# tyb311/TCCT

Measured on AMD Instinct MI355X. Metric: OCT B-scans/sec fwd+bwd(+clip+AdamW), stc_tt bs=8 1x800x1100, higher is better.
Workload: dtype bf16; 1 GPU; stc_tt --los=di bs=8/GPU 1x800x1100 (net tensors 3x800x1104); global_batch=8, parallelism=dp1, ranks=1, grad_allreduce=none, slowest_step=88

## Files before the change

### include/tcct_hip.h

```cpp
#ifndef TCCT_HIP_H
#define TCCT_HIP_H
#include <stdint.h>
#ifdef __cplusplus
extern "C" {
#endif

typedef void* tcct_stream_t;

enum { TCCT_F32 = 0, TCCT_BF16 = 1 };
enum { TCCT_ACT_NONE = 0, TCCT_ACT_LRELU = 1, TCCT_ACT_HSWISH = 2, TCCT_ACT_GELU = 3, TCCT_ACT_SIGMOID = 4,
       TCCT_ACT_ABS = 5 };
enum { TCCT_CRIT_DICE = 0, TCCT_CRIT_DICE2 = 1, TCCT_CRIT_IOU = 2, TCCT_CRIT_MSE = 3 };
enum { TCCT_MCRIT_DICE = 0, TCCT_MCRIT_DICE2 = 1, TCCT_MCRIT_IOU = 2, TCCT_MCRIT_CE = 3 };

int tcct_version(void);
const char* tcct_last_error(void);
int tcct_set_outputs_prezeroed(int on);

int tcct_image_to_nhwc4(const float* img, void* out, int N, int Csrc, int H, int Wsrc, int Wdst, int dtype,
                        tcct_stream_t stream);
int tcct_u8_gather2d(const uint8_t* src, uint8_t* dst, int N, int SH, int SW, int C, int sy0, int sx0, int sh, int sw, int DH, int DW,
                     int dy0, int dx0, int dh, int dw, int flipy, int flipx, int mul, int div, int fill, tcct_stream_t stream);
int tcct_onehot_to_index(const int64_t* onehot, uint8_t* lab, int N, int C, int64_t HW, tcct_stream_t stream);
int tcct_labels_to_u8(const int64_t* lab, uint8_t* out, int N, int H, int Wsrc, int Wdst, tcct_stream_t stream);
// ... 59 lines not shown
                           int pre_act, int act, int dtype, tcct_stream_t stream);
int tcct_bn2_add_act_bwd_reduce(const void* xa, const void* xb, const void* dy, int64_t M, int C, const float* mean_rstdA,
                                const float* abA, const float* mean_rstdB, const float* abB, int pre_act, int act, double* sums,
                                int dtype, tcct_stream_t stream);
int tcct_bn2_add_act_bwd_apply(const void* xa, const void* xb, const void* dy, void* dxa, void* dxb, int64_t M, int C,
                               const float* mean_rstdA, const float* abA, const float* mean_rstdB, const float* abB,
                               const double* sums, int pre_act, int act, float* dgammaA, float* dbetaA, float* dgammaB,
                               float* dbetaB, int dtype, tcct_stream_t stream);

int tcct_layernorm_fwd(const void* x, void* y, int64_t M, int C, const float* gamma, const float* beta, float eps,
                       float* mean_rstd , int dtype, tcct_stream_t stream);
int tcct_layernorm_bwd(const void* x, const void* dy, void* dx, int64_t M, int C, const float* gamma,
                       const float* mean_rstd, float* dgamma, float* dbeta, int dtype, tcct_stream_t stream);
int tcct_layernorm_bwd_add(const void* x, const void* dy, const void* res, void* dx, int64_t M, int C, const float* gamma,
                           const float* mean_rstd, float* dgamma, float* dbeta, int dtype, tcct_stream_t stream);

int tcct_conv2d_fwd(const void* x, const float* w, const float* bias, void* y, int N, int H, int W, int Cin,
                    int Cin_w, int Cout, int KH, int KW, int stride, int padh, int padw, int in_dtype, int out_dtype,
                    tcct_stream_t stream);
int tcct_conv2d_dgrad(const void* dy, const float* w, void* dx, int N, int H, int W, int Cin, int Cout, int KH,
                      int KW, int padh, int padw, int dy_dtype, int dx_dtype, tcct_stream_t stream);
int tcct_conv2d_wgrad(const void* x, const void* dy, float* dw, float* dbias, int N, int H, int W, int Cin,
                      int Cin_w, int Cout, int KH, int KW, int stride, int padh, int padw, int x_dtype, int dy_dtype,
                      tcct_stream_t stream);

int tcct_conv32f_pack_weights(const float* w, float* wp, int KH, int KW, int transposed, tcct_stream_t stream);
int tcct_conv32f_fwd(const float* x, const float* wp, const float* bias, const float* yadd, float* y, int N, int H, int W, int KH, int KW, int PH,
                     int PW, tcct_stream_t stream);
int tcct_conv32f_wgrad(const float* x, const float* dy, float* dw, float* dbias, int N, int H, int W, int KH, int KW, int PH, int PW,
                       tcct_stream_t stream);
int tcct_conv32f_pack_weights_sub(const float* w, float* wp, int KH, int KW, int transposed, int cin_total, int o_off, int i_off, tcct_stream_t stream);
int tcct_conv32f_fwd_strided(const float* x, const float* wp, const float* bias, float* y, int N, int H, int W, int KH, int KW, int PH, int PW, int xs,
                             int xo, int ys, int yo, int accumulate, tcct_stream_t stream);
int tcct_conv32f_wgrad_strided(const float* x, const float* dy, float* dw, float* dbias, int N, int H, int W, int KH, int KW, int PH, int PW, int xs,
                               int xo, int ds, int dof, int ldi, int o_off, int i_off, tcct_stream_t stream);
int tcct_pwf_fwd(const float* x, const float* w, const float* bias, float* y, int64_t M, int K, int N, int transposed, tcct_stream_t stream);
int tcct_pwf_wgrad(const float* x, const float* dy, float* dw, float* dbias, int64_t M, int K, int N, tcct_stream_t stream);
int tcct_conv32_pack_weights(const float* w, void* wp, int KH, int KW, int transposed, tcct_stream_t stream);
int tcct_conv32_pack_weights_multi(const void* desc, int n, tcct_stream_t stream);
int tcct_conv32_pack_weights_both(const float* w, void* wp2, int KH, int KW, tcct_stream_t stream);
int tcct_conv32_fwd(const void* x, const void* wp, const float* bias, void* y, int N, int H, int W, int KH, int KW, int PH,
                    int PW, tcct_stream_t stream);

int tcct_conv32_fwd_bnstats(const void* x, const void* wp, const float* bias, void* y, int N, int H, int W, int KH, int KW, int PH,
                            int PW, double* stats, int pre_act, tcct_stream_t stream);
int tcct_conv32_fwd_affine(const void* x, const void* wp, const float* bias, void* y, int N, int H, int W, int KH, int KW,
                           int PH, int PW, const float* ab, int pre_act, int post_act, tcct_stream_t stream);
int tcct_pw_fwd_affine(const void* x, const float* w, const float* bias, void* y, int64_t M, int K, int N, const float* ab,
                       int pre_act, int post_act, int out_dtype, tcct_stream_t stream);
int tcct_pw_fwd_affine_residual(const void* x, const float* w, const float* bias, const float* ab, const void* res, void* y, int64_t M, int K, int N,
                                tcct_stream_t stream);
int tcct_pw_fwd_cat2_affine(const void* x1, const void* x2, const float* w, const float* bias, const float* ab, int post_act, void* y, int64_t M, int K, int N,
                            tcct_stream_t stream);
int tcct_pw_fwd_xaff_affine_residual(const void* y_prev, const float* ab_prev, const float* w, const float* bias, const float* ab, const void* res, void* y,
                                     int64_t M, int K, int N, tcct_stream_t stream);
int tcct_conv32_fwd_add(const void* x, const void* wp, const float* bias, const void* res, void* y, int N, int H, int W, int KH, int KW,
                        int PH, int PW, tcct_stream_t stream);
int tcct_conv32_chain33(const void* x, const void* wp1, const float* bias1, void* mid, const void* wp2, const float* bias2, void* y,
                        const void* res, int N, int H, int W, double* stats, tcct_stream_t stream);
int tcct_conv32_pack_weights_sub(const float* w, void* wp, int KH, int KW, int transposed, int cin_total, int o_off, int i_off,
                                 tcct_stream_t stream);
int tcct_conv32_fwd_strided(const void* x, const void* wp, const float* bias, void* y, int N, int H, int W, int KH, int KW, int PH,
                            int PW, int xs, int xo, int ys, int yo, int accumulate, tcct_stream_t stream);
int tcct_conv32_fwd_strided_bnstats(const void* x, const void* wp, const float* bias, void* y, int N, int H, int W, int KH, int KW, int PH,
                                    int PW, int xs, int xo, int ys, int yo, int accumulate, double* stats, int pre_act, tcct_stream_t stream);
int tcct_conv32_fwd_strided_affine(const void* x, const void* wp, const float* bias, void* y, int N, int H, int W, int KH, int KW, int PH, int PW, int xs,
                                   int xo, int ys, int yo, const float* ab, int pre_act, int post_act, tcct_stream_t stream);
int64_t tcct_conv32_wgrad_mode(int mode);
int64_t tcct_conv32_fwd_mode(int mode);
int tcct_conv32_wgrad_strided(const void* x, const void* dy, float* dw, float* dbias, int N, int H, int W, int KH, int KW, int PH,
                              int PW, int xs, int xo, int ds, int dof, int cin_total, int o_off, int i_off, tcct_stream_t stream);
int tcct_conv32x64_fwd33(const void* x, const void* wp, int wps, const float* bias, void* y, int N, int H, int W, double* stats, int pre_act, int force,
                         tcct_stream_t stream);
int tcct_conv32x64_wgrad33(const void* x, const void* dy, float* dw, float* dbias, int N, int H, int W, int force, tcct_stream_t stream);
int tcct_conv64x32_dgrad33(const void* dy, const void* wp_t, int wps, void* dx, int N, int H, int W, int force, tcct_stream_t stream);
int tcct_conv32_wgrad(const void* x, const void* dy, float* dw, float* dbias, int N, int H, int W, int KH, int KW, int PH,
                      int PW, tcct_stream_t stream);
int tcct_conv32_bwd3x3(const void* x, const void* dy, const void* wp_t, const void* dskip, void* dx, float* dw, float* dbias, int N, int H,
                       int W, tcct_stream_t stream);

int tcct_pw_fwd(const void* x, const float* w, const float* bias, void* y, int64_t M, int K, int N, int transposed,
                int out_dtype, tcct_stream_t stream);
int tcct_pw_wgrad(const void* x, const void* dy, float* dw, float* dbias, int64_t M, int K, int N, tcct_stream_t stream);
int tcct_pw_bwd(const void* x, const void* dy, const float* w, const void* res, void* dx, float* dw, float* dbias, int64_t M, int K, int N,
                tcct_stream_t stream);
int tcct_pw_bwd_cat2(const void* x1, const void* x2, const void* dy, const float* w, void* dx1, void* dx2, float* dw, int64_t M, int K, int N,
                     tcct_stream_t stream);
int tcct_pw_bwd_residual2(const void* x, const void* dy, const float* w, const void* res, void* dx_sum, void* dx_plain, float* dw, float* dbias,
                          int64_t M, int K, int N, tcct_stream_t stream);
int64_t tcct_pw_bwd_bn_supported(int K, int N, int post, int red_post, int split);
int tcct_pw_bwd_bn(const void* x, const void* x2, const void* dz, const void* y, const float* coef, int post, const float* w, const void* res,
                   void* dx, void* dx2, float* dw, float* dbias, int64_t M, int K, int N, const void* y_prev, const float* ab_prev,
                   int red_post, double* sums_prev, tcct_stream_t stream);
int tcct_pw_bwd_bn_sums(const void* x, const void* x2, const void* dz, const void* y, const double* sums, int raw, const float* mean_rstd,
                        const float* ab, float* dgamma, float* dbeta, int post, const float* w, const void* res, void* dx, void* dx2, float* dw,
                        float* dbias, int64_t M, int K, int N, const void* y_prev, const float* ab_prev, int red_post, double* sums_prev,
                        tcct_stream_t stream);
int tcct_pw_wgrad_strided(const void* x, const void* dy, int64_t ldy, float* dw, float* dbias, int64_t M, int K, int N,
                          tcct_stream_t stream);
int tcct_pw_fwd_residual(const void* x, const float* w, const float* bias, const void* res, const float* scale, int64_t per_sample,
                         void* y, void* y_plain, int64_t M, int K, int N, tcct_stream_t stream);
int tcct_pw_fwd_bnstats_xaff(const void* y_prev, const float* ab_prev, const float* w, const float* bias, void* y, int64_t M, int K, int N, double* stats,
                             tcct_stream_t stream);
int tcct_pw_bwd_bn_sums_xaff(const void* y_prev, const float* ab_prev, const void* dz, const void* y, const double* sums, int raw, const float* mean_rstd,
                             const float* ab, float* dgamma, float* dbeta, const float* w, const void* res, void* dx, float* dw, float* dbias, int64_t M,
                             int K, int N, int red_post, double* sums_prev, tcct_stream_t stream);
int tcct_pw_fwd_gelu_residual(const void* x1, const float* w, const float* bias, const void* res, const float* scale, int64_t per_sample, void* y,
                              int64_t M, int K, int N, tcct_stream_t stream);
int tcct_pw_bwd_residual2_sum(const void* x, const void* dy_a, const void* dy_b, const float* w, const void* res, void* dx_sum, void* dx_plain, float* dw,
                              float* dbias, int64_t M, int K, int N, tcct_stream_t stream);
int tcct_pw_bwd_lnb(const void* x, const void* dy, const float* w, const void* t, const float* mean_rstd, const float* gamma, const void* res, void* dt,
                    float* dw, float* dbias, float* dgamma, float* dbeta, int64_t M, int K, int N, tcct_stream_t stream);
int tcct_pw_bwd_gelu(const void* x1, const void* dy, const float* w, void* dx1, float* dw, float* dbias, int64_t M, int K, int N, tcct_stream_t stream);
int tcct_pw_dgrad_residual(const void* dy, const float* w, const void* res, void* dx_sum, void* dx_plain, int64_t M, int Nout, int K,
                           tcct_stream_t stream);
int tcct_pw_fwd_cat2(const void* x1, const void* x2, int K1, const float* w, const float* bias, void* y, int64_t M, int K, int N,
                     double* stats, int pre_act, tcct_stream_t stream);
int tcct_pw_fwd_f32_upadd(const void* x, const float* w, const float* bias, float* y, int B, int uH, int uW, int K, int N, const float* up, tcct_stream_t stream);
int tcct_pw_dgrad_split2(const void* dy, const float* w, void* dx1, void* dx2, int K1, int64_t M, int Nout, int K, tcct_stream_t stream);
int tcct_pw_bwd_cat2_bias(const void* x1, const void* x2, const void* dy, const float* w, void* dx1, void* dx2, float* dw, float* dbias, int64_t M,
                          int K, int N, tcct_stream_t stream);
int tcct_tail_compose(const float* w1, const float* b1, const float* w2, const float* b2, float* wc, float* c, tcct_stream_t stream);
int tcct_tail_compose_bwd(const float* w1, const float* b1, const float* w2, const float* dwc, const float* dc, float* dw1, float* db1, float* dw2,
                          float* db2, tcct_stream_t stream);
int tcct_tail_compose3(const float* w1, const float* b1, const float* w2, const float* b2, const float* w3, const float* b3, int C, float* wcc, float* wa,
                       float* wb, float* ccc, tcct_stream_t stream);
int tcct_tail_compose3_bwd(const float* w1, const float* b1, const float* w2, const float* b2, const float* w3, int C, const float* dwa, const float* dwb,
                           const float* dccc, float* dw1, float* db1, float* dw2, float* db2, float* dw3, float* db3, tcct_stream_t stream);
int tcct_pw_fwd_cat2_f32(const void* x1, const void* x2, int K1, const float* w, const float* bias, float* y, int64_t M, int K, int N, tcct_stream_t stream);
int tcct_head_compose(const float* wt, const float* bt, const float* wa, const float* ba, int C, float* wh, float* ch, tcct_stream_t stream);
int tcct_head_compose_bwd(const float* wt, const float* bt, const float* wa, int C, const float* dwh, const float* dch, float* dwt, float* dbt,
                          float* dwa, float* dba, tcct_stream_t stream);
int tcct_pw_wgrad_cat2(const void* x1, const void* x2, int K1, const void* dy, float* dw, float* dbias, int64_t M, int K, int N,
                       tcct_stream_t stream);
int tcct_pw_fwd_bnstats(const void* x, const float* w, const float* bias, void* y, int64_t M, int K, int N, double* stats, int pre_act,
                        tcct_stream_t stream);

int tcct_im2col3x3_c3(const void* x4, void* out, int N, int H, int W, int stride, int dtype, tcct_stream_t stream);
int tcct_c3_fwd(const void* x4, const float* w, const float* bias, void* y, int B, int H, int W, int stride, double* stats, int stat_pre,
                const float* ab, int pre_act, int post_act, tcct_stream_t stream);
int tcct_c3_wgrad(const void* x4, const void* dy, float* dw, float* dbias, int B, int H, int W, int stride, tcct_stream_t stream);
int tcct_c3_bn_fwd_train(const void* x4, const float* w, const float* bias, void* z, int B, int H, int W, int stride, double* sums,
                         const float* gamma, const float* beta, float eps, float momentum, float* running_mean, float* running_var,
                         int64_t* num_batches_tracked, float* mean_rstd, float* ab, int post_act, tcct_stream_t stream);
int tcct_c3_bn_fwd_eval(const void* x4, const float* w, const float* bias, void* z, int B, int H, int W, int stride, const float* ab, int post_act,
                        tcct_stream_t stream);
int tcct_c3_bn_bwd_reduce(const void* x4, const float* w, const float* bias, const void* dz, int B, int H, int W, int stride, const float* ab,
                          double* raw, int post_act, tcct_stream_t stream);
int tcct_c3_bn_bwd_wgrad(const void* x4, const float* w, const float* bias, const void* dz, int B, int H, int W, int stride, const float* coef,
                         float* dw, float* dbias, int post_act, tcct_stream_t stream);
int64_t tcct_c3_bn_bwd_prefetch(int tiles_ahead);
int tcct_c3_bn_bwd_onepass(const void* x4, const float* w, const float* bias, const void* dz, int B, int H, int W, int stride, const float* mean_rstd,
                           const float* ab, float* work, double* sums, float* dw, float* dbias, float* dgamma, float* dbeta, int post_act, tcct_stream_t stream);
int tcct_pw_wgrad_smalln(const void* x, const void* dy, float* dw, float* dbias, int64_t M, int K, int N, int x_dtype,
                         int dy_dtype, tcct_stream_t stream);

int tcct_stream_copy(const void* src, void* dst, int64_t nbytes, tcct_stream_t stream);

int64_t tcct_kernel_census(int which, int reset);
int tcct_marker(int id, tcct_stream_t stream);

int tcct_dwconv3x3_fwd(const void* x, const float* w, const float* bias, void* y, int N, int H, int W, int C,
                       int stride, int add_input, int dtype, tcct_stream_t stream);
int tcct_dwconv3x3_fwd_bnstats(const void* x, const float* w, const float* bias, void* y, int N, int H, int W, int C, int stride,
                               int add_input, double* stats, int dtype, tcct_stream_t stream);
int tcct_dwconv3x3_dgrad(const void* dy, const float* w, void* dx, int N, int H, int W, int C, int stride,
// ... 182 lines not shown
```

### tcct_amd/csrc/common.h

```cpp
#pragma once
#include <hip/hip_runtime.h>
#include <hip/hip_bf16.h>
#include <stdint.h>
#include <stdio.h>
#include "../../include/tcct_hip.h"

typedef __hip_bfloat16 bf16;

void tcct_set_error(const char* fmt, ...);
enum { TCCT_CENSUS_CHAIN33 = 0, TCCT_CENSUS_WGRADK_STREAM = 1, TCCT_CENSUS_WGRAD33_STREAM = 2, TCCT_CENSUS_FWD33_STREAM = 3,
       TCCT_CENSUS_PW_FWD = 4, TCCT_CENSUS_PW_FWD_NT0 = 4, TCCT_CENSUS_PW_FWD2 = 10, TCCT_CENSUS_PW_BWD = 11, TCCT_CENSUS_PW_WGRAD = 12,
       TCCT_CENSUS_PW_WGRAD_SMALLN = 13, TCCT_CENSUS_PW_WGRAD_SMALLN_MFMA = 14, TCCT_CENSUS_PWF_FWD = 15, TCCT_CENSUS_PWF_WGRAD = 16,
       TCCT_CENSUS_DW_FWD_S1 = 17, TCCT_CENSUS_DW_FWD_S2 = 18, TCCT_CENSUS_DW_FWD_CPT4 = 19, TCCT_CENSUS_DW_DGRAD_S2 = 20, TCCT_CENSUS_DW_WGRAD = 21,
       TCCT_CENSUS_DW_WGRAD_CPT2 = 22, TCCT_CENSUS_N = 24 };
void tcct_census_hit(int which);
int tcct_skip_zero_fill();

#define TCCT_CHECK(cond, ...)                                   \
    do {                                                        \
        if (!(cond)) {                                          \
            tcct_set_error(__VA_ARGS__);                        \
            return -1;                                          \
        }                                                       \
    } while (0)

#define TCCT_LAUNCH_OK()                                                        \
    do {                                                                        \
        hipError_t e__ = hipGetLastError();                                     \
        if (e__ != hipSuccess) {                                                \
            tcct_set_error("%s: launch failed: %s", __func__, hipGetErrorString(e__)); \
            return -2;                                                          \
        }                                                                       \
        return 0;                                                               \
    } while (0)

#define TCCT_DISPATCH(dtype, ...)                                               \
    do {                                                                        \
        if ((dtype) == TCCT_F32) { typedef float T; __VA_ARGS__; }              \
        else if ((dtype) == TCCT_BF16) { typedef bf16 T; __VA_ARGS__; }         \
        else { tcct_set_error("%s: bad dtype %d", __func__, (int)(dtype)); return -1; } \
    } while (0)

static inline int tcct_grid(int64_t work_items, int block, int cap = 256 * 16) {
    int64_t g = (work_items + block - 1) / block;
    if (g < 1) g = 1;
    if (g > cap) g = cap;
    return (int)g;
}

template <auto Kern, int MAX_LDS_BYTES, typename... Args>
static void tcct_launch(dim3 grid, dim3 block, size_t lds, hipStream_t st, Args... args) {
    static const hipError_t once = hipFuncSetAttribute((const void*)Kern, hipFuncAttributeMaxDynamicSharedMemorySize, MAX_LDS_BYTES);
    (void)once;
    hipLaunchKernelGGL(Kern, grid, block, lds, st, args...);
}

__device__ __forceinline__ float ldf(const float* p) { return *p; }
__device__ __forceinline__ float ldf(const bf16* p) { return __bfloat162float(*p); }
__device__ __forceinline__ void stf(float* p, float v) { *p = v; }
__device__ __forceinline__ void stf(bf16* p, float v) { *p = __float2bfloat16(v); }

struct f4 { float v[4]; };

__device__ __forceinline__ f4 ld4(const float* p) {
    float4 t = *reinterpret_cast<const float4*>(p);
    f4 r; r.v[0] = t.x; r.v[1] = t.y; r.v[2] = t.z; r.v[3] = t.w; return r;
}
__device__ __forceinline__ f4 ld4(const bf16* p) {
    uint2 t = *reinterpret_cast<const uint2*>(p);
    f4 r;
    r.v[0] = __uint_as_float(t.x << 16); r.v[1] = __uint_as_float(t.x & 0xffff0000u);
    r.v[2] = __uint_as_float(t.y << 16); r.v[3] = __uint_as_float(t.y & 0xffff0000u);
    return r;
}
__device__ __forceinline__ void st4(float* p, const f4& a) {
    *reinterpret_cast<float4*>(p) = make_float4(a.v[0], a.v[1], a.v[2], a.v[3]);
}
typedef __bf16 bf16x2_hw __attribute__((ext_vector_type(2)));
typedef float f32x2_hw __attribute__((ext_vector_type(2)));
__device__ __forceinline__ uint32_t pack_bf16x2(float lo, float hi) {
    const f32x2_hw v = {lo, hi};
    return __builtin_bit_cast(uint32_t, __builtin_convertvector(v, bf16x2_hw));
}
__device__ __forceinline__ void st4(bf16* p, const f4& a) {
    uint2 t; t.x = pack_bf16x2(a.v[0], a.v[1]); t.y = pack_bf16x2(a.v[2], a.v[3]);
    *reinterpret_cast<uint2*>(p) = t;
}
__device__ __forceinline__ f4 f4zero() { f4 r; r.v[0] = r.v[1] = r.v[2] = r.v[3] = 0.f; return r; }

template <int VEC> __device__ __forceinline__ void ldv(const float* p, float* o) {
    if (VEC == 1) { o[0] = *p; return; }
#pragma unroll
    for (int j = 0; j < VEC / 4; ++j) {
        const float4 t = *reinterpret_cast<const float4*>(p + 4 * j);
        o[4 * j] = t.x; o[4 * j + 1] = t.y; o[4 * j + 2] = t.z; o[4 * j + 3] = t.w;
    }
}
// ... 162 lines not shown
```

### tcct_amd/csrc/pw_mfma.hip

```cpp
#include "common.h"
#include "c3_geom.h"
#include <cstdlib>

typedef __attribute__((ext_vector_type(8))) __bf16 bf16x8;
typedef __attribute__((ext_vector_type(16))) float f32x16;
typedef __attribute__((ext_vector_type(4))) short s16x4;
typedef __attribute__((ext_vector_type(8))) short s16x8;

#define PWB 256

__device__ __forceinline__ void st_out4(bf16* p, float a, float b, float c, float d) {
    uint2 o; o.x = pack_bf16x2(a, b); o.y = pack_bf16x2(c, d);
    *reinterpret_cast<uint2*>(p) = o;
}
__device__ __forceinline__ void st_out4(float* p, float a, float b, float c, float d) {
    *reinterpret_cast<float4*>(p) = make_float4(a, b, c, d);
}


struct PwUp { const float* p; int uH, uW, Ho, Wo; float sh, sw; uint32_t m_howo, m_wo; };
struct PwSplit { const bf16* x2; int K1; void* y2; int N1; const bf16* res; const float* rscale; int64_t per_sample; bf16* yplain; C3Geom c3; PwUp up; };
template <int NT, typename Tout, bool STATS, bool AFF, bool C3 = false>
__global__ void __launch_bounds__(PWB, 2)
k_pw_fwd(const bf16* __restrict__ x, const float* __restrict__ w, const float* __restrict__ bias, Tout* __restrict__ y,
// ... 551 lines not shown
                for (int j = 0; j < 8; ++j) bsum[ct] += (float)f.a[ct][j];
        }
#pragma unroll
        for (int kt = 0; kt < KTB; ++kt)
#pragma unroll
            for (int ct = 0; ct < NT; ++ct) acc[ct][kt] = __builtin_amdgcn_mfma_f32_32x32x16_bf16(f.a[ct], f.b[kt], acc[ct][kt], 0, 0, 0);
    };
    const int64_t tiles = (M + PW_P - 1) / PW_P;
    int64_t tile = blockIdx.x;
    if (C3)
        for (int i = tid; i < PW_P * 2; i += PWB) *reinterpret_cast<uint4*>(sX + (i >> 1) * SX + (6 + (i & 1)) * 16) = make_uint4(0, 0, 0, 0);
    if (tile < tiles) prefetch(tile);
    for (; tile < tiles; tile += gridDim.x) {
        __syncthreads();
        if (C3) {
#pragma unroll
            for (int j = 0; j < 3; ++j)
                if (xsl[j] >= 0) *reinterpret_cast<uint4*>(sX + (tid & 127) * SX + (xsl[j] & 255) * 16) = px[j];
        } else
#pragma unroll
        for (int j = 0; j < PW_XS; ++j)
            if (xsl[j] >= 0) *reinterpret_cast<uint4*>(sX + (xsl[j] >> 8) * SX + (xsl[j] & 255) * 16) = px[j];
#pragma unroll
        for (int j = 0; j < DSN; ++j)
            if (dsl[j] >= 0) *reinterpret_cast<uint4*>(sD + (dsl[j] >> 8) * SD + (dsl[j] & 255) * 16) = pd[j];
        __syncthreads();
        if (C3 || tile + gridDim.x < tiles) prefetch(tile + gridDim.x);
        WF f0, f1;
        load_chunk(f0, wave);
        load_chunk(f1, wave + 4);
        __builtin_amdgcn_sched_barrier(0);
        mma_chunk(f0);
        mma_chunk(f1);
        __builtin_amdgcn_sched_barrier(0);
    }
    __syncthreads();
    float* red = reinterpret_cast<float*>(smem);
    for (int turn = 0; turn < 4; ++turn) {
        if (wave == turn) {
#pragma unroll
            for (int ct = 0; ct < NT; ++ct)
#pragma unroll
                for (int kt = 0; kt < KTB; ++kt)
#pragma unroll
                    for (int k = 0; k < 16; ++k) {
                        const int co = ct * 32 + (k & 3) + 8 * (k >> 2) + 4 * hh;
                        float* dst = &red[co * (KTB * 32) + kt * 32 + r];
                        *dst = turn == 0 ? acc[ct][kt][k] : *dst + acc[ct][kt][k];
                    }
        }
        __syncthreads();
    }
    for (int i = tid; i < NT * 32 * KTB * 32; i += PWB) {
        const int co = i / (KTB * 32), cl = i - co * (KTB * 32);
        if (C3) {
            if (cl < 48 && ((cl >> 2) & 3) < 3 && (cl & 3) < 3) atomicAdd(&dw[co * 27 + (cl & 3) * 9 + (cl >> 4) * 3 + ((cl >> 2) & 3)], red[i]);
        }
        else
        if (co < N && ci_base + cl < K) atomicAdd(&dw[(int64_t)co * K + ci_base + cl], red[i]);
    }
    if (dbias && blockIdx.y == 0) {
#pragma unroll
        for (int ct = 0; ct < NT; ++ct) {
            float s = bsum[ct] + __shfl_xor(bsum[ct], 32, 64);
            if (lane < 32 && ct * 32 + r < N) atomicAdd(&dbias[ct * 32 + r], s);
        }
    }
}

static int pw_wgrad_impl(const void* x, const void* x2, int K1, const void* dy, float* dw, float* dbias, int64_t M, int K, int N, tcct_stream_t stream,
                         int64_t ldy);
extern "C" int tcct_pw_wgrad(const void* x, const void* dy, float* dw, float* dbias, int64_t M, int K, int N, tcct_stream_t stream) {
    return pw_wgrad_impl(x, nullptr, 0, dy, dw, dbias, M, K, N, stream, 0);
}
extern "C" int tcct_pw_wgrad_cat2(const void* x1, const void* x2, int K1, const void* dy, float* dw, float* dbias, int64_t M, int K, int N,
                                  tcct_stream_t stream) {
    TCCT_CHECK(x2 != nullptr && K1 % 32 == 0 && K1 > 0 && K1 < K, "pw_wgrad_cat2: K1=%d must be a multiple of 32 inside (0, K)", K1);
    return pw_wgrad_impl(x1, x2, K1, dy, dw, dbias, M, K, N, stream, 0);
}
extern "C" int tcct_pw_wgrad_strided(const void* x, const void* dy, int64_t ldy, float* dw, float* dbias, int64_t M, int K, int N,
                                     tcct_stream_t stream) {
    return pw_wgrad_impl(x, nullptr, 0, dy, dw, dbias, M, K, N, stream, ldy);
}
static int pw_wgrad_impl(const void* x, const void* x2, int K1, const void* dy, float* dw, float* dbias, int64_t M, int K, int N, tcct_stream_t stream,
                         int64_t ldy) {
    if (ldy == 0) ldy = N;
    TCCT_CHECK(ldy >= N && ldy % 8 == 0, "pw_wgrad: ldy=%lld must be a multiple of 8 and >= N=%d", (long long)ldy, N);
    TCCT_CHECK(K % 32 == 0 && N % 32 == 0 && K >= 32 && N >= 32 && N <= 160 && K <= 1024, "pw_wgrad: unsupported K=%d N=%d", K, N);
    hipStream_t st = (hipStream_t)stream;
    const int NT = N / 32, ktiles = K / 32;
    const int KTB = (ktiles % 2 == 0 && NT <= 2) ? 2 : 1;
    const int gy = ktiles / KTB;
    TCCT_CHECK(!x2 || K1 % (KTB * 32) == 0, "pw_wgrad_cat2: K1=%d must be a multiple of %d for this shape", K1, KTB * 32);
    if (!tcct_skip_zero_fill() && hipMemsetAsync(dw, 0, sizeof(float) * (size_t)N * K, st) != hipSuccess) { tcct_set_error("pw_wgrad: memset failed"); return -2; }
    if (dbias && !tcct_skip_zero_fill() && hipMemsetAsync(dbias, 0, sizeof(float) * N, st) != hipSuccess) { tcct_set_error("pw_wgrad: memset failed"); return -2; }
    const int SX = KTB == 1 ? 64 : 192;
    const int SD = 2 * N + ((NT & 1) ? 0 : 64);
    size_t lds = (size_t)PW_P * (SX + SD);
    size_t red = (size_t)NT * 32 * KTB * 32 * 4;
    if (red > lds) lds = red;
    const int64_t tiles = (M + PW_P - 1) / PW_P;
    int per_cu = (int)((160 * 1024) / (lds + 512));
    if (per_cu > 2) per_cu = 2;
    if (per_cu < 1) per_cu = 1;
    int gx = 256 * per_cu / gy;
    if (gx < 64) gx = 64;
    if (tiles <= 1024) { int small = 128 / gy; if (small < 16) small = 16; if (gx > small) gx = small; }
    if (gx > tiles) gx = (int)tiles;
    if (gx < 1) gx = 1;
    tcct_census_hit(TCCT_CENSUS_PW_WGRAD);
#define WL(NTV, KV) tcct_launch<k_pw_wgrad<NTV, KV>, 160 * 1024>(dim3(gx, gy), dim3(PWB), lds, st, (const bf16*)x, (const bf16*)dy, dw, dbias, M, K, N, SX, SD, (const bf16*)x2, K1, ldy, C3Geom{})
    if (KTB == 2) { switch (NT) { case 1: WL(1, 2); break; default: WL(2, 2); break; } }
    else { switch (NT) { case 1: WL(1, 1); break; case 2: WL(2, 1); break; case 3: WL(3, 1); break; case 4: WL(4, 1); break; default: WL(5, 1); break; } }
#undef WL
    TCCT_LAUNCH_OK();
}


extern "C" int tcct_c3_wgrad(const void* x4, const void* dy, float* dw, float* dbias, int B, int H, int W, int stride, tcct_stream_t stream) {
    TCCT_CHECK(stride == 1 || stride == 2, "c3_wgrad: stride %d", stride);
    const int Ho = (H - 1) / stride + 1, Wo = (W - 1) / stride + 1;
    const int64_t M = (int64_t)B * Ho * Wo, inb = (int64_t)B * H * W * 8;
    TCCT_CHECK(M > 0 && M * 64 < (1ll << 31) && inb < (1ll << 31), "c3_wgrad: image too large for 32-bit byte offsets (B=%d H=%d W=%d)", B, H, W);
    hipStream_t st = (hipStream_t)stream;
    if (!tcct_skip_zero_fill() && hipMemsetAsync(dw, 0, sizeof(float) * 32 * 27, st) != hipSuccess) { tcct_set_error("c3_wgrad: memset failed"); return -2; }
    if (dbias && !tcct_skip_zero_fill() && hipMemsetAsync(dbias, 0, sizeof(float) * 32, st) != hipSuccess) { tcct_set_error("c3_wgrad: memset failed"); return -2; }
    const int SX = 192, SD = 64;
    const size_t lds = (size_t)PW_P * (SX + SD);
    const int64_t tiles = (M + PW_P - 1) / PW_P;
    int gx = (int)(tiles / 48 < 256 ? 256 : (tiles / 48 > 1024 ? 1024 : tiles / 48));
    if (gx > tiles) gx = (int)tiles;
    auto magic = [](uint32_t d) { return d == 1 ? 0xffffffffu : (uint32_t)((1ull << 32) / d); };
    hipLaunchKernelGGL((k_pw_wgrad<1, 2, true>), dim3(gx, 1), dim3(PWB), lds, st, (const bf16*)x4, (const bf16*)dy, dw, dbias, M, 64, 32, SX, SD,
                       (const bf16*)nullptr, 0, (int64_t)32,
                       C3Geom{H, W, Ho, Wo, stride, (uint32_t)inb, (Wo + 31) / 32, magic((uint32_t)((Wo + 31) / 32)), magic((uint32_t)Ho), magic((uint32_t)(Ho * Wo)), magic((uint32_t)Wo)});
    TCCT_LAUNCH_OK();
}


#define PB_P 128

__device__ __forceinline__ u32x4 gelu8(u32x4 v) {
    u32x4 o;
#pragma unroll
    for (int k = 0; k < 4; ++k)
        o[k] = pack_bf16x2(act_c<TCCT_ACT_GELU>(__uint_as_float(v[k] << 16)), act_c<TCCT_ACT_GELU>(__uint_as_float(v[k] & 0xffff0000u)));
    return o;
}
__device__ __forceinline__ float gelu_grad1(float x) { float c, p; gauss_cdf_pdf(x, c, p); return c + x * p; }
template <int KIND> __device__ __forceinline__ u32x4 affine8(u32x4 v, const float* __restrict__ a, const float* __restrict__ b) {
    const float4 a0 = *reinterpret_cast<const float4*>(a), a1 = *reinterpret_cast<const float4*>(a + 4);
    const float4 b0 = *reinterpret_cast<const float4*>(b), b1 = *reinterpret_cast<const float4*>(b + 4);
    const float aa[8] = {a0.x, a0.y, a0.z, a0.w, a1.x, a1.y, a1.z, a1.w}, bb[8] = {b0.x, b0.y, b0.z, b0.w, b1.x, b1.y, b1.z, b1.w};
    u32x4 o;
#pragma unroll
    for (int k = 0; k < 4; ++k)
        o[k] = pack_bf16x2(act_c<KIND>(aa[2 * k] * __uint_as_float(v[k] << 16) + bb[2 * k]),
                           act_c<KIND>(aa[2 * k + 1] * __uint_as_float(v[k] & 0xffff0000u) + bb[2 * k + 1]));
    return o;
}
struct PwBnBwd { const bf16* y; const float* coef; const bf16* yprev; const float* abprev; double* sums_prev;
                 const double* sums; int raw; const float* mean_rstd; const float* ab; float* dgamma; float* dbeta; };
template <int KIND> __device__ __forceinline__ float pw_act_grad(float u) {
    if (KIND == TCCT_ACT_HSWISH) return u < -3.f ? 0.f : (u <= 3.f ? (2.f * u + 3.f) * (1.f / 6.f) : 1.f);
    return 1.f;
}
template <int NT, int KT, bool SPLIT = false, int BNP = -1, int REDP = -1, bool GX = false, int XAP = -1, bool LNB = false, bool DY2 = false>
__global__ void __launch_bounds__(PWB, 2)
k_pw_bwd(const bf16* __restrict__ x, const bf16* __restrict__ dy, const float* __restrict__ w, const bf16* __restrict__ res,
         bf16* __restrict__ dx, bf16* __restrict__ dx_plain, float* __restrict__ dw, float* __restrict__ dbias, int64_t M, PwBnBwd bn) {
    constexpr int K = 32 * KT, N = 32 * NT;
    constexpr bool BN = BNP >= 0, RED = REDP >= 0;
    constexpr int SX = 64 * KT + ((KT & 1) ? 0 : 64), SD = 64 * NT + ((NT & 1) ? 0 : 64);
    constexpr int SW = 2 * N + 16;
    constexpr int XS = K / 16, DS = N / 16;
    extern __shared__ __attribute__((aligned(16))) unsigned char smem[];
    unsigned char* sX = smem;
    unsigned char* sD = sX + PB_P * SX;
    unsigned char* sW = sD + PB_P * SD;
    unsigned char* sS = sW + ((K * SW + 15) & ~15);
    float* sC = reinterpret_cast<float*>(sS + 4 * 2560);
    float* sP = sC + (BN ? 5 * N : 0);
    const int tid = threadIdx.x, lane = tid & 63, wave = tid >> 6;
    const int r = lane & 31, hh = lane >> 5;
    for (int i = tid; i < N * K; i += PWB) {
        const int n = i / K, k = i - n * K;
        *reinterpret_cast<bf16*>(sW + k * SW + n * 2) = __float2bfloat16(w[i]);
    }
    if (BN) {
        if (bn.coef) { for (int i = tid; i < 5 * N; i += PWB) sC[i] = bn.coef[i]; }
        else if (tid < N) {
            const int c = tid;
            const double mu = bn.mean_rstd[c], rs = bn.mean_rstd[N + c];
// ... 995 lines not shown
```

Before: 431.6 B-scans/s.

## Add single-pass pointwise wgrad kernel that reads each input tile once

Adds a new pointwise weight-gradient kernel for specific (N, K) shapes. Each 512-thread block stages all K input channels and all N output-gradient channels for a 128-pixel tile in LDS. Every wave then accumulates its share of the 32x32 output tiles with MFMA, so x and dy are read once instead of once per K-tile column of the grid. It is chosen when the streamed bytes are large relative to the weight size, and uses a sqrt-based persistent grid with double-buffered register prefetch. The cost is a large per-thread accumulator count and fewer blocks, which can limit occupancy and add atomic traffic at the end.

```diff
diff --git a/include/tcct_hip.h b/include/tcct_hip.h
--- a/include/tcct_hip.h
+++ b/include/tcct_hip.h
@@ -165,6 +165,7 @@
 int tcct_pw_fwd(const void* x, const float* w, const float* bias, void* y, int64_t M, int K, int N, int transposed,
                 int out_dtype, tcct_stream_t stream);
 int tcct_pw_wgrad(const void* x, const void* dy, float* dw, float* dbias, int64_t M, int K, int N, tcct_stream_t stream);
+int64_t tcct_pw_wgrad_mode(int mode);
 int tcct_pw_bwd(const void* x, const void* dy, const float* w, const void* res, void* dx, float* dw, float* dbias, int64_t M, int K, int N,
                 tcct_stream_t stream);
 int tcct_pw_bwd_cat2(const void* x1, const void* x2, const void* dy, const float* w, void* dx1, void* dx2, float* dw, int64_t M, int K, int N,
diff --git a/tcct_amd/csrc/common.h b/tcct_amd/csrc/common.h
--- a/tcct_amd/csrc/common.h
+++ b/tcct_amd/csrc/common.h
@@ -12,7 +12,9 @@
        TCCT_CENSUS_PW_FWD = 4, TCCT_CENSUS_PW_FWD_NT0 = 4, TCCT_CENSUS_PW_FWD2 = 10, TCCT_CENSUS_PW_BWD = 11, TCCT_CENSUS_PW_WGRAD = 12,
        TCCT_CENSUS_PW_WGRAD_SMALLN = 13, TCCT_CENSUS_PW_WGRAD_SMALLN_MFMA = 14, TCCT_CENSUS_PWF_FWD = 15, TCCT_CENSUS_PWF_WGRAD = 16,
        TCCT_CENSUS_DW_FWD_S1 = 17, TCCT_CENSUS_DW_FWD_S2 = 18, TCCT_CENSUS_DW_FWD_CPT4 = 19, TCCT_CENSUS_DW_DGRAD_S2 = 20, TCCT_CENSUS_DW_WGRAD = 21,
-       TCCT_CENSUS_DW_WGRAD_CPT2 = 22, TCCT_CENSUS_N = 24 };
+       TCCT_CENSUS_DW_WGRAD_CPT2 = 22,
+       TCCT_CENSUS_PW_WGRAD_ONCE = 23,
+       TCCT_CENSUS_N = 24 };
 void tcct_census_hit(int which);
 int tcct_skip_zero_fill();
 
diff --git a/tcct_amd/csrc/pw_mfma.hip b/tcct_amd/csrc/pw_mfma.hip
--- a/tcct_amd/csrc/pw_mfma.hip
+++ b/tcct_amd/csrc/pw_mfma.hip
@@ -657,6 +657,135 @@
                                      tcct_stream_t stream) {
     return pw_wgrad_impl(x, nullptr, 0, dy, dw, dbias, M, K, N, stream, ldy);
 }
+
+#define PWO_P 128
+#define PWO_B 512
+#define PWO_RATIO 32.0
+#define PWO_MIN_RATIO 150.0
+template <int NT, int KT>
+__global__ void __launch_bounds__(PWO_B)
+k_pw_wgrad_once(const bf16* __restrict__ x, const bf16* __restrict__ x2, int KT1, const bf16* __restrict__ dy, int64_t ldy, float* __restrict__ dw,
+                float* __restrict__ dbias, int64_t M) {
+    constexpr int K = 32 * KT, N = 32 * NT;
+    constexpr int SX = 64 * KT + ((KT & 1) ? 0 : 64), SD = 64 * NT + ((NT & 1) ? 0 : 64);
+    constexpr int DC = N / 8;
+    constexpr int ACC = (NT * KT + 7) / 8;
+    static_assert(PWO_P * 4 == PWO_B, "one 32-channel tile of 128 pixels = one 16-byte slot per thread");
+    extern __shared__ __attribute__((aligned(16))) unsigned char smem[];
+    unsigned char* sX = smem;
+    unsigned char* sD = smem + PWO_P * SX;
+    const int tid = threadIdx.x, lane = tid & 63, wave = __builtin_amdgcn_readfirstlane(tid >> 6);
+    const int r = lane & 31, hh = lane >> 5;
+    const int K1 = 32 * KT1, K2 = K - K1;
+    const uint32_t ldb = (uint32_t)ldy * 2u;
+    const __amdgpu_buffer_rsrc_t rx = __builtin_amdgcn_make_buffer_rsrc((void*)x, 0, (uint32_t)(M * K1 * 2), 0x00020000);
+    const __amdgpu_buffer_rsrc_t rx2 = __builtin_amdgcn_make_buffer_rsrc((void*)(K2 ? x2 : x), 0, (uint32_t)(M * K2 * 2), 0x00020000);
+    const __amdgpu_buffer_rsrc_t rd = __builtin_amdgcn_make_buffer_rsrc((void*)dy, 0, (uint32_t)(((M - 1) * ldy + N) * 2), 0x00020000);
+    int xdst[KT], ddst[NT], dpix[NT];
+    uint32_t dsrc[NT];
+#pragma unroll
+    for (int j = 0; j < KT; ++j) {
+        const bool second = j >= KT1;
+        const int xc = (second ? K2 : K1) >> 3, q = tid + (second ? j - KT1 : j) * PWO_B, p = q / xc, c = q - p * xc;
+        xdst[j] = p * SX + (second ? K1 * 2 : 0) + c * 16;
+    }
+#pragma unroll
+    for (int j = 0; j < NT; ++j) {
+        const int q = tid + j * PWO_B, p = q / DC, c = q - p * DC;
+        ddst[j] = p * SD + c * 16; dpix[j] = p; dsrc[j] = (uint32_t)p * ldb + (uint32_t)c * 16u;
+    }
+    f32x16 acc[ACC];
+    float bsum[ACC];
+#pragma unroll
+    for (int a = 0; a < ACC; ++a) {
+        bsum[a] = 0.f;
+#pragma unroll
+        for (int k = 0; k < 16; ++k) acc[a][k] = 0.f;
+    }
+    const int64_t tiles = (M + PWO_P - 1) / PWO_P;
+    u32x4 px[KT], pd[NT];
+    auto prefetch = [&](int64_t t) {
+        const bool live = t < tiles;
+        const int64_t m0 = t * PWO_P;
+        const int rows = live ? (int)(M - m0 < PWO_P ? M - m0 : PWO_P) : 0;
+        const uint32_t b1 = (uint32_t)(m0 * K1 * 2), b2 = (uint32_t)(m0 * K2 * 2), bd = (uint32_t)m0 * ldb;
+        const uint32_t dead = live ? 0u : 0x80000000u;
+#pragma unroll
+        for (int j = 0; j < KT; ++j) {
+            const bool first = j < KT1;
+            const uint32_t off = (first ? b1 : b2) + (uint32_t)(tid + (first ? j : j - KT1) * PWO_B) * 16u;
+            px[j] = __builtin_amdgcn_raw_buffer_load_b128(first ? rx : rx2, off | dead, 0, 0);
+        }
+#pragma unroll
+        for (int j = 0; j < NT; ++j) pd[j] = __builtin_amdgcn_raw_buffer_load_b128(rd, dpix[j] < rows ? bd + dsrc[j] : 0x80000000u, 0, 0);
+    };
+    const int li = lane & 15, lq = li >> 2, lpp = li & 3, lg = lane >> 4;
+    const int lrow = 8 * (lg >> 1) + lq, lcol = (16 * (lg & 1) + 4 * lpp) * 2;
+    const unsigned char* lbX = sX + lrow * SX + lcol;
+    const unsigned char* lbD = sD + lrow * SD + lcol;
+    auto tr2 = [&](const unsigned char* p, int stride) {
+        s16x4 lo = __builtin_amdgcn_ds_read_tr16_b64_v4i16((__attribute__((address_space(3))) s16x4*)p);
+        s16x4 hi = __builtin_amdgcn_ds_read_tr16_b64_v4i16((__attribute__((address_space(3))) s16x4*)(p + 4 * stride));
+        s16x8 v = __builtin_shufflevector(lo, hi, 0, 1, 2, 3, 4, 5, 6, 7);
+        return __builtin_bit_cast(bf16x8, v);
+    };
+    int64_t tile = blockIdx.x;
+    prefetch(tile);
+    for (; tile < tiles; tile += gridDim.x) {
+        __syncthreads();
+#pragma unroll
+        for (int j = 0; j < KT; ++j) *reinterpret_cast<u32x4*>(sX + xdst[j]) = px[j];
+#pragma unroll
+        for (int j = 0; j < NT; ++j) *reinterpret_cast<u32x4*>(sD + ddst[j]) = pd[j];
+        __syncthreads();
+        prefetch(tile + gridDim.x);
+#pragma unroll
+        for (int a = 0; a < ACC; ++a) {
+            const int ti = wave + 8 * a;
+            if (ti < NT * KT) {
+                const int ct = ti / KT, kt = ti - ct * KT;
+                const float bw = kt == 0 ? 1.f : 0.f;
+#pragma unroll
+                for (int ch = 0; ch < PWO_P / 16; ++ch) {
+                    const bf16x8 fa = tr2(lbD + ch * 16 * SD + 64 * ct, SD);
+                    const bf16x8 fb = tr2(lbX + ch * 16 * SX + 64 * kt, SX);
+                    float s = 0.f;
+#pragma unroll
+                    for (int j = 0; j < 8; ++j) s += (float)fa[j];
+                    bsum[a] += bw * s;
+                    acc[a] = __builtin_amdgcn_mfma_f32_32x32x16_bf16(fa, fb, acc[a], 0, 0, 0);
+                }
+            }
+        }
+    }
+#pragma unroll
+    for (int a = 0; a < ACC; ++a) {
+        const int ti = wave + 8 * a;
+        if (ti < NT * KT) {
+            const int ct = ti / KT, kt = ti - ct * KT;
+#pragma unroll
+            for (int k = 0; k < 16; ++k) {
+                const int co = ct * 32 + (k & 3) + 8 * (k >> 2) + 4 * hh;
+                atomicAdd(&dw[(int64_t)co * K + kt * 32 + r], acc[a][k]);
+            }
+            if (dbias && kt == 0) {
+                const float sb = bsum[a] + __shfl_xor(bsum[a], 32, 64);
+                if (lane < 32) atomicAdd(&dbias[ct * 32 + r], sb);
+            }
+        }
+    }
+}
+typedef void (*PwOnceLaunch)(dim3, dim3, size_t, hipStream_t, const bf16*, const bf16*, int, const bf16*, int64_t, float*, float*, int64_t);
+struct PwOnceRow { int nt, kt; PwOnceLaunch launch; };
+#define PWO_ROW(NT, KT) {NT, KT, tcct_launch<k_pw_wgrad_once<NT, KT>, 160 * 1024>}
+static const PwOnceRow pw_once_table[] = { PWO_ROW(4, 6), PWO_ROW(5, 8), PWO_ROW(5, 10), PWO_ROW(5, 5), PWO_ROW(5, 4) };
+#undef PWO_ROW
+static int g_pw_wgrad_mode = 0;
+extern "C" int64_t tcct_pw_wgrad_mode(int mode) {
+    const int prev = g_pw_wgrad_mode;
+    if (mode >= 0 && mode <= 2) g_pw_wgrad_mode = mode;
+    return prev;
+}
 static int pw_wgrad_impl(const void* x, const void* x2, int K1, const void* dy, float* dw, float* dbias, int64_t M, int K, int N, tcct_stream_t stream,
                          int64_t ldy) {
     if (ldy == 0) ldy = N;
@@ -684,6 +813,22 @@
     if (gx > tiles) gx = (int)tiles;
     if (gx < 1) gx = 1;
     tcct_census_hit(TCCT_CENSUS_PW_WGRAD);
+    const PwOnceRow* once = nullptr;
+    const double bytes = (double)M * (K + N) * 2.0, kn4 = (double)K * N * 4.0;
+    if ((g_pw_wgrad_mode == 2 || (g_pw_wgrad_mode == 0 && bytes >= PWO_MIN_RATIO * kn4)) && (M + PWO_P) * (K > ldy ? K : ldy) * 2 < (1LL << 31))
+        for (const PwOnceRow& r : pw_once_table)
+            if (r.nt == NT && r.kt == ktiles) once = &r;
+    if (once) {
+        tcct_census_hit(TCCT_CENSUS_PW_WGRAD_ONCE);
+        const size_t olds = (size_t)PWO_P * ((64 * ktiles + ((ktiles & 1) ? 0 : 64)) + (64 * NT + ((NT & 1) ? 0 : 64)));
+        const int64_t otiles = (M + PWO_P - 1) / PWO_P;
+        int64_t ob = (int64_t)__builtin_sqrt(bytes * PWO_RATIO / kn4);
+        if (ob > 256) ob = 256;
+        if (ob > otiles) ob = otiles;
+        if (ob < 1) ob = 1;
+        once->launch(dim3((unsigned)ob), dim3(PWO_B), olds, st, (const bf16*)x, (const bf16*)x2, x2 ? K1 / 32 : ktiles, (const bf16*)dy, ldy, dw, dbias, M);
+        TCCT_LAUNCH_OK();
+    }
 #define WL(NTV, KV) tcct_launch<k_pw_wgrad<NTV, KV>, 160 * 1024>(dim3(gx, gy), dim3(PWB), lds, st, (const bf16*)x, (const bf16*)dy, dw, dbias, M, K, N, SX, SD, (const bf16*)x2, K1, ldy, C3Geom{})
     if (KTB == 2) { switch (NT) { case 1: WL(1, 2); break; default: WL(2, 2); break; } }
     else { switch (NT) { case 1: WL(1, 1); break; case 2: WL(2, 1); break; case 3: WL(3, 1); break; case 4: WL(4, 1); break; default: WL(5, 1); break; } }
```

New measurement: 433.1 B-scans/s (median of 6 runs). No clear change (+0.3%).
